# uingei/hevc

Hardware: AMD Instinct MI355X
Metric: encoded 1080p30 frames/sec/GPU; PSNR-Y parity vs libx265 at matched bitrate (higher is better)
Workload: dtype u8

## Files before the change

hevc_amd/csrc/device.hip:

```cpp
#include "device.h"
#include "md5.h"

#include <cstdio>
#include <cstring>
#include <vector>

namespace mihevc {

__host__ __device__ static inline size_t round16(size_t v) { return (v + 15) & ~(size_t)15; }

__device__ __forceinline__ int xcd_remap(int b, int n)
{
    int chunk = (n + 7) >> 3;
    return (b & 7) * chunk + (b >> 3);
}

template <typename T> __global__ __launch_bounds__(NT, 5) void k_me_search(const InterArgs<T> *args, int n_ctu, int list)
{
    extern __shared__ __align__(16) unsigned char smem[];
    const int ctu = xcd_remap(blockIdx.x, n_ctu);
    if (ctu >= n_ctu) return;
    MeShared<T> &s = *reinterpret_cast<MeShared<T> *>(smem);
    uint8_t *win = smem + round16(sizeof(MeShared<T>));
    GpuExec ex;
    if (list) {
        const InterArgs<T> a = list1_view(args[blockIdx.y]);
        me_search_program<T>(ex, s, win, a, ctu);
    } else me_search_program<T>(ex, s, win, args[blockIdx.y], ctu);
}

template <typename T> __global__ __launch_bounds__(NT, 4) void k_inter_ctu(const InterArgs<T> *args, int n_ctu)
{
    extern __shared__ __align__(16) unsigned char smem[];
    const int ctu = xcd_remap(blockIdx.x, n_ctu);
    if (ctu >= n_ctu) return;
    const InterArgs<T> &a = args[blockIdx.y];
    const int R = a.prm.me_range;
    InterShared<T> &s = *reinterpret_cast<InterShared<T> *>(smem);
    size_t off = round16(sizeof(InterShared<T>));
    T *wy = reinterpret_cast<T *>(smem + off);
    off += round16(((size_t)mc_win_y(R) * mc_win_y_stride(R) + 16) * sizeof(T));
    T *wu = reinterpret_cast<T *>(smem + off);
    off += round16(((size_t)mc_win_c(R) * mc_win_c_stride(R) + 16) * sizeof(T));
    T *wv = reinterpret_cast<T *>(smem + off);
    GpuExec ex;
    inter_ctu_program<T>(ex, s, wy, wu, wv, a, ctu);
}

template <typename T> __global__ __launch_bounds__(NT, 3) void k_inter_ctu_b(const InterArgs<T> *args, int n_ctu)
{
    extern __shared__ __align__(16) unsigned char smem[];
    const int ctu = xcd_remap(blockIdx.x, n_ctu);
    if (ctu >= n_ctu) return;
    const InterArgs<T> &a = args[blockIdx.y];
    const int R = a.prm.me_range;
    InterShared<T> &s = *reinterpret_cast<InterShared<T> *>(smem);
    size_t off = round16(sizeof(InterShared<T>));
    T *wy = reinterpret_cast<T *>(smem + off);
    off += round16(((size_t)mc_win_y(R) * mc_win_y_stride(R) + 16) * sizeof(T));
    T *wu = reinterpret_cast<T *>(smem + off);
    off += round16(((size_t)mc_win_c(R) * mc_win_c_stride(R) + 16) * sizeof(T));
    T *wv = reinterpret_cast<T *>(smem + off);
    off += round16(((size_t)mc_win_c(R) * mc_win_c_stride(R) + 16) * sizeof(T));
    BiShared *b = reinterpret_cast<BiShared *>(smem + off);
    GpuExec ex;
    inter_ctu_program<T, GpuExec, true>(ex, s, wy, wu, wv, a, ctu, b);
}

#ifndef INTRA_OCC
#define INTRA_OCC 3
#endif
template <typename T> __global__ __launch_bounds__(NT, (sizeof(T) == 1 ? INTRA_OCC : 2)) void k_intra_plan(const IntraArgs<T> *args, int n_ctu)
{
    extern __shared__ __align__(16) unsigned char smem[];
    const int ctu = xcd_remap(blockIdx.x, n_ctu);
    if (ctu >= n_ctu) return;
    const IntraArgs<T> &a = args[blockIdx.y];
    IntraShared<T> &s = *reinterpret_cast<IntraShared<T> *>(smem);
    GpuExec ex;
    intra_plan_program<T>(ex, s, a, ctu % a.ctus_w, ctu / a.ctus_w);
}

template <typename T> __global__ __launch_bounds__(NT, 2) void k_intra_diag(const IntraArgs<T> *args, int diagonal, int rows_per_tile)
{
    extern __shared__ __align__(16) unsigned char smem[];
    const IntraArgs<T> &a = args[blockIdx.y];
    const int tcn = a.prm.tile_cols > 1 ? a.prm.tile_cols : 1, trn = a.prm.tile_rows > 1 ? a.prm.tile_rows : 1;
    const int tile = (int)blockIdx.x / rows_per_tile, r = (int)blockIdx.x % rows_per_tile;
    if (tile >= tcn * trn) return;
    const int tx = tile % tcn, ty = tile / tcn;
    const int cx0 = tile_bd(tx, tcn, a.ctus_w), cx1 = tile_bd(tx + 1, tcn, a.ctus_w), cy0 = tile_bd(ty, trn, a.ctus_h), cy1 = tile_bd(ty + 1, trn, a.ctus_h);
    const int cy = cy0 + r, cx = cx0 + diagonal - 2 * r;
    if (cy >= cy1 || cx < cx0 || cx >= cx1) return;
    IntraShared<T> &s = *reinterpret_cast<IntraShared<T> *>(smem);
    GpuExec ex;
    intra_code_program<T>(ex, s, a, cx, cy, true);
}

template <typename T> __global__ __launch_bounds__(256) void k_lowres(const PreArgs<T> *args)
// ... 209 lines not shown
        i -= ncp;
        if (i < ncp) pad_border_quad<T>(a.out[2], a.w >> 1, a.h >> 1, PAD_C, i, a.halo_top >> 1, a.halo_bottom >> 1);
        return;
    }
    b -= n_pad_blocks;
    if (b < n_low_blocks) { lowres_sample<T>(pre[g], b * 256 + (int)threadIdx.x); return; }
    if (threadIdx.x == 0) {
        CostParams c = p.prm[g];
        ea[g].prm = c; sa[g].prm = c;
        c.tile_cols = p.p_tile_cols; c.tile_rows = p.p_tile_rows;
        ia[g].prm = c;
    }
    if (threadIdx.x < 4) sa[g].sse[threadIdx.x] = 0;
}

template <typename T> hipError_t launch_prep_p_step(hipStream_t st, const SaoArgs<T> *prev, const PreArgs<T> *pre, IntraArgs<T> *ia, InterArgs<T> *ea, SaoArgs<T> *sa,
                                                    const StepParams &p, int w, int h, int batch)
{
    if (batch > MAX_LANES) return hipErrorInvalidValue;
    const int n_pad = prev ? (pad_border_quads(w, h, PAD_Y) + 2 * pad_border_quads(w >> 1, h >> 1, PAD_C) + 255) / 256 : 0;
    const int n_low = pre ? (2 * (w >> 2) * (h >> 2) + 255) / 256 : 0;
    hipLaunchKernelGGL(k_prep_p_step<T>, dim3((unsigned)(n_pad + n_low + 1), (unsigned)batch), dim3(256), 0, st, prev, n_pad, pre, n_low, ia, ea, sa, p);
    return hipGetLastError();
}
template <typename T> hipError_t launch_begin_p_step(hipStream_t st, IntraArgs<T> *ia, InterArgs<T> *ea, SaoArgs<T> *sa, const StepParams &p, int batch)
{
    if (batch > MAX_LANES) return hipErrorInvalidValue;
    hipLaunchKernelGGL(k_begin_p_step<T>, dim3((unsigned)batch), dim3(64), 0, st, ia, ea, sa, p);
    return hipGetLastError();
}
template <typename T> hipError_t launch_frame_sse(hipStream_t st, const SaoArgs<T> *d_args, int batch)
{
    hipLaunchKernelGGL(k_frame_sse<T>, dim3(256, (unsigned)batch), dim3(256), 0, st, d_args);
    return hipGetLastError();
}
template <typename K> static hipError_t ensure_smem(K kernel, size_t bytes)
{
    if (bytes <= 48 * 1024) return hipSuccess;
    return hipFuncSetAttribute(reinterpret_cast<const void *>(kernel), hipFuncAttributeMaxDynamicSharedMemorySize, (int)bytes);
}

template <typename T> hipError_t launch_me_search(hipStream_t st, const InterArgs<T> *d_args, int n_ctu, int batch, int R, int list)
{
    size_t smem = round16(sizeof(MeShared<T>)) + round16((size_t)me_win_elems(R));
    hipError_t e = ensure_smem(k_me_search<T>, smem);
    if (e != hipSuccess) return e;
    dim3 grid((unsigned)(((n_ctu + 7) >> 3) << 3), (unsigned)batch);
    hipLaunchKernelGGL(k_me_search<T>, grid, dim3(NT), smem, st, d_args, n_ctu, list);
    return hipGetLastError();
}

template <typename T> hipError_t launch_inter_ctu(hipStream_t st, const InterArgs<T> *d_args, int n_ctu, int batch, int R)
{
    size_t smem = round16(sizeof(InterShared<T>)) + round16(((size_t)mc_win_y(R) * mc_win_y_stride(R) + 16) * sizeof(T)) +
                  2 * round16(((size_t)mc_win_c(R) * mc_win_c_stride(R) + 16) * sizeof(T));
    hipError_t e = ensure_smem(k_inter_ctu<T>, smem);
    if (e != hipSuccess) return e;
    dim3 grid((unsigned)(((n_ctu + 7) >> 3) << 3), (unsigned)batch);
    hipLaunchKernelGGL(k_inter_ctu<T>, grid, dim3(NT), smem, st, d_args, n_ctu);
    return hipGetLastError();
}

template <typename T> hipError_t launch_inter_ctu_b(hipStream_t st, const InterArgs<T> *d_args, int n_ctu, int batch, int R)
{
    size_t smem = round16(sizeof(InterShared<T>)) + round16(((size_t)mc_win_y(R) * mc_win_y_stride(R) + 16) * sizeof(T)) +
                  2 * round16(((size_t)mc_win_c(R) * mc_win_c_stride(R) + 16) * sizeof(T)) + round16(sizeof(BiShared));
    hipError_t e = ensure_smem(k_inter_ctu_b<T>, smem);
    if (e != hipSuccess) return e;
    dim3 grid((unsigned)(((n_ctu + 7) >> 3) << 3), (unsigned)batch);
    hipLaunchKernelGGL(k_inter_ctu_b<T>, grid, dim3(NT), smem, st, d_args, n_ctu);
    return hipGetLastError();
}

template <typename T> hipError_t launch_intra_picture(hipStream_t st, const IntraArgs<T> *d_args, int ctus_w, int ctus_h, int batch, int tile_cols, int tile_rows, hipEvent_t after_plan)
{
    size_t smem = round16(sizeof(IntraShared<T>));
    hipError_t e = ensure_smem(k_intra_plan<T>, smem);
    if (e != hipSuccess) return e;
    e = ensure_smem(k_intra_diag<T>, smem);
    if (e != hipSuccess) return e;
    if (tile_cols < 1) tile_cols = 1;
    if (tile_rows < 1) tile_rows = 1;
    const int n_ctu = ctus_w * ctus_h;
    hipLaunchKernelGGL(k_intra_plan<T>, dim3((unsigned)(((n_ctu + 7) >> 3) << 3), (unsigned)batch), dim3(NT), smem, st, d_args, n_ctu);
    if (after_plan) { e = hipEventRecord(after_plan, st); if (e != hipSuccess) return e; }
    const int colw = (ctus_w + tile_cols - 1) / tile_cols, rowh = (ctus_h + tile_rows - 1) / tile_rows;
    for (int d = 0; d <= (colw - 1) + 2 * (rowh - 1); d++)
        hipLaunchKernelGGL(k_intra_diag<T>, dim3((unsigned)(tile_cols * tile_rows * rowh), (unsigned)batch), dim3(NT), smem, st, d_args, d, rowh);
    return hipGetLastError();
}

template <typename T> hipError_t launch_pre_search(hipStream_t st, const PreArgs<T> *d_args, int w, int h, int n_ctu, int batch, bool with_lowres)
{
    const int n = 2 * (w >> 2) * (h >> 2);
    if (with_lowres) hipLaunchKernelGGL(k_lowres<T>, dim3((unsigned)((n + 255) / 256), (unsigned)batch), dim3(256), 0, st, d_args);
    hipLaunchKernelGGL(k_pre_search<T>, dim3((unsigned)n_ctu, (unsigned)batch), dim3(NT), 0, st, d_args, n_ctu);
    return hipGetLastError();
}

template <typename T> __global__ __launch_bounds__(256) void k_lowres_src(const PreArgs<T> *args)
{
    const PreArgs<T> &a = args[blockIdx.y];
    const int i = (int)(blockIdx.x * 256 + threadIdx.x);
    if (i < (a.w >> 2) * (a.h >> 2)) lowres_sample<T>(a, i);
}
template <typename T> hipError_t launch_pre_search_chunk(hipStream_t st, const PreArgs<T> *d_args, int w, int h, int n_ctu, int n_pictures)
{
    if (n_pictures <= 0) return hipSuccess;
    const int n = (w >> 2) * (h >> 2);
    hipLaunchKernelGGL(k_lowres_src<T>, dim3((unsigned)((n + 255) / 256), (unsigned)n_pictures), dim3(256), 0, st, d_args);
    hipLaunchKernelGGL(k_pre_search<T>, dim3((unsigned)n_ctu, (unsigned)n_pictures), dim3(NT), 0, st, d_args, n_ctu);
    return hipGetLastError();
// ... 558 lines not shown
```

hevc_amd/csrc/kernels/common.h:

```cpp
#pragma once
#include <stdint.h>

#if defined(__HIPCC__)
#include <hip/hip_runtime.h>
#define DEV __device__ __forceinline__
#define HD __host__ __device__
#define HDI __host__ __device__ inline
#define DEVCONST __device__ const
#define MIHEVC_GPU 1
#else
#define DEV inline
#define HD
#define HDI inline
#define DEVCONST static const
#define MIHEVC_GPU 0
#endif

#include "../../../include/mihevc.h"

namespace mihevc {

constexpr int CTU = 32;
constexpr int CTU_LOG2 = 5;
constexpr int PAD_Y = 80;
// ... 237 lines not shown
DEV void copy_window(T *lds, int ls, const T *plane, int pstride, int ox, int oy, int w, int h, int lo_x, int hi_x, int lo_y, int hi_y, int tid)
{
    constexpr int per = 4 / (int)sizeof(T);
    constexpr int CH = 6;
    const int dpr = w / per, col = tid & 31, rg = tid >> 5;
    for (int d = col; d < dpr; d += 32) {
        const int x = clip3(lo_x, hi_x - (per - 1), ox + d * per);
        for (int r0 = rg; r0 < h; r0 += CH * (NT / 32)) {
            uint32_t v[CH];
#pragma unroll
            for (int k = 0; k < CH; k++) {
                const int r = r0 + k * (NT / 32);
                if (r < h) v[k] = load_u32(plane + (ptrdiff_t)clip3(lo_y, hi_y, oy + r) * pstride + x);
            }
#pragma unroll
            for (int k = 0; k < CH; k++) {
                const int r = r0 + k * (NT / 32);
                if (r < h) __builtin_memcpy(__builtin_assume_aligned(lds + r * ls + d * per, 4), &v[k], 4);
            }
        }
    }
}

template <typename T>
DEV void load_ctu_source(T *dst, const Plane<const T> (&src)[3], int x0, int y0, int w, int h, int tid)
{
    constexpr int per = 4 / (int)sizeof(T);
    if (x0 + CTU <= w && y0 + CTU <= h) {
        constexpr int ND = 1536 / per, IT = (ND + NT - 1) / NT;
        uint32_t v[IT];
#pragma unroll
        for (int k = 0; k < IT; k++) {
            const int d = tid + k * NT;
            if (d < ND) {
                const int i = d * per, pl = i < 1024 ? 0 : 1 + ((i - 1024) >> 8), kk = pl ? (i - 1024) & 255 : i, x = pl ? kk & 15 : kk & 31, y = pl ? kk >> 4 : kk >> 5;
                v[k] = load_u32(src[pl].p + (size_t)((pl ? y0 >> 1 : y0) + y) * src[pl].stride + (pl ? x0 >> 1 : x0) + x);
            }
        }
#pragma unroll
        for (int k = 0; k < IT; k++) {
            const int d = tid + k * NT;
            if (d < ND) __builtin_memcpy(__builtin_assume_aligned(dst + d * per, 4), &v[k], 4);
        }
        return;
    }
    for (int i = tid; i < 1536; i += NT) {
        int pl, x, y;
        if (i < 1024) { pl = 0; x = i & 31; y = i >> 5; } else { int k = i - 1024; pl = 1 + (k >> 8); k &= 255; x = k & 15; y = k >> 4; }
        const int gx = (pl ? x0 >> 1 : x0) + x, gy = (pl ? y0 >> 1 : y0) + y, pw = pl ? w >> 1 : w, ph = pl ? h >> 1 : h;
        dst[i] = (gx < pw && gy < ph) ? src[pl].p[(size_t)gy * src[pl].stride + gx] : (T)0;
    }
}

DEV int opaque_zero()
{
    int z = 0;
#if MIHEVC_GPU
    asm volatile("" : "+v"(z));
#endif
    return z;
}
DEV uint32_t load_u32_aligned(const void *p)
{
    uint32_t v;
    __builtin_memcpy(&v, __builtin_assume_aligned(p, 4), 4);
    return v;
}
DEV void store_u32_aligned(void *p, uint32_t v) { __builtin_memcpy(__builtin_assume_aligned(p, 4), &v, 4); }
DEV void store4(uint8_t *p, int v0, int v1, int v2, int v3) { store_u32_aligned(p, (uint32_t)v0 | (uint32_t)v1 << 8 | (uint32_t)v2 << 16 | (uint32_t)v3 << 24); }
DEV void store4(uint16_t *p, int v0, int v1, int v2, int v3)
{
    store_u32_aligned(p, (uint32_t)v0 | (uint32_t)v1 << 16);
    store_u32_aligned(p + 2, (uint32_t)v2 | (uint32_t)v3 << 16);
}
DEV void store4(int16_t *p, int v0, int v1, int v2, int v3)
{
    store_u32_aligned(p, ((uint32_t)v0 & 0xffffu) | (uint32_t)v1 << 16);
    store_u32_aligned(p + 2, ((uint32_t)v2 & 0xffffu) | (uint32_t)v3 << 16);
}
DEV void load_row15(const uint8_t *base, int idx, int (&px)[15])
{
    const int off = idx & 3;
    const uint8_t *p = base + (idx - off);
    uint32_t d[5];
#pragma unroll
    for (int k = 0; k < 5; k++) d[k] = load_u32_aligned(p + 4 * k);
    uint32_t r[4];
#pragma unroll
    for (int k = 0; k < 4; k++) r[k] = align_bytes(d[k + 1], d[k], off);
#pragma unroll
    for (int i = 0; i < 15; i++) px[i] = (int)((r[i >> 2] >> (8 * (i & 3))) & 255);
}
DEV void load_row15(const uint16_t *base, int idx, int (&px)[15])
{
    const int off = idx & 1;
    const uint16_t *p = base + (idx - off);
    uint32_t d[8];
#pragma unroll
    for (int k = 0; k < 8; k++) d[k] = load_u32_aligned(p + 2 * k);
    uint32_t r[8];
#pragma unroll
    for (int k = 0; k < 7; k++) r[k] = align_bytes(d[k + 1], d[k], 2 * off);
    r[7] = align_bytes(0, d[7], 2 * off);
#pragma unroll
    for (int i = 0; i < 15; i++) px[i] = (int)((r[i >> 1] >> (16 * (i & 1))) & 65535);
}
// ... 89 lines not shown
    int s = 0;
#pragma unroll
    for (int x = 0; x < 8; x++) {
#pragma unroll
        for (int st = 1; st < 8; st <<= 1)
#pragma unroll
            for (int i = 0; i < 8; i++)
                if (!(i & st)) { int p = m[i][x], q = m[i + st][x]; m[i][x] = p + q; m[i + st][x] = p - q; }
#pragma unroll
        for (int i = 0; i < 8; i++) if (x || i) s += iabs(m[i][x]);
    }
    return (s + 2) >> 2;
}

#if MIHEVC_GPU
#ifdef MIHEVC_PHASE_PROF
__device__ unsigned long long g_phase_prof[8 * 1024 * 3];
#endif
struct GpuExec {
    static DEV int lane_id()
    {
        int t = (int)threadIdx.x;
        asm volatile("" : "+v"(t));
        return t;
    }
#ifdef MIHEVC_PHASE_PROF
    template <class F> DEV void phase(F &&f, int line = __builtin_LINE(), const char *file = __builtin_FILE())
    {
        int len = 0;
        while (file[len]) len++;
        const int fid = ((int)file[len - 3] + 2 * (int)file[len - 4] + 3 * (int)file[len - 6]) & 7;
        const int slot = (fid * 1024 + (line & 1023)) * 3;
        const unsigned long long t0 = __builtin_amdgcn_s_memtime();
        f(lane_id());
        const unsigned long long t1 = __builtin_amdgcn_s_memtime();
        __syncthreads();
        if (threadIdx.x == 0) {
            const unsigned long long t2 = __builtin_amdgcn_s_memtime();
            atomicAdd(&g_phase_prof[slot], t2 - t0);
            atomicAdd(&g_phase_prof[slot + 1], t1 - t0);
            atomicAdd(&g_phase_prof[slot + 2], 1ull);
        }
    }
#else
    template <class F> DEV void phase(F &&f)
    {
        f(lane_id());
        __syncthreads();
    }
#endif
    template <class F> DEV void wave_step(F &&f)
    {
        f(lane_id());
        __builtin_amdgcn_fence(__ATOMIC_SEQ_CST, "wavefront");
        __builtin_amdgcn_wave_barrier();
    }
    DEV void atomic_add(int *p, int v) { atomicAdd(p, v); }
    DEV void atomic_add(unsigned *p, unsigned v) { atomicAdd(p, v); }
    DEV void atomic_add(unsigned long long *p, unsigned long long v) { atomicAdd(p, v); }
    DEV void atomic_or(unsigned *p, unsigned v) { atomicOr(p, v); }
    DEV void atomic_and(unsigned *p, unsigned v) { atomicAnd(p, v); }
    DEV void atomic_min(unsigned long long *p, unsigned long long v) { atomicMin(p, v); }
    DEV unsigned long long peek(const unsigned long long *p) { return __atomic_load_n(p, __ATOMIC_RELAXED); }
    DEV void atomic_add_global(unsigned long long *p, unsigned long long v) { atomicAdd(p, v); }
};
#endif
struct SeqExec {
    int order = 0;
    unsigned long long rnd = 0x2545F4914F6CDD1Dull;
    template <class F> void run(F &&f)
    {
        if (order == 0) { for (int t = 0; t < NT; t++) f(t); return; }
        if (order == 1) { for (int t = NT - 1; t >= 0; t--) f(t); return; }
        int perm[NT];
        for (int i = 0; i < NT; i++) perm[i] = i;
        for (int i = NT - 1; i > 0; i--) {
            rnd ^= rnd << 13; rnd ^= rnd >> 7; rnd ^= rnd << 17;
            int j = (int)((rnd >> 33) % (unsigned)(i + 1)), tmp = perm[i];
            perm[i] = perm[j]; perm[j] = tmp;
        }
        for (int i = 0; i < NT; i++) f(perm[i]);
    }
    template <class F> void phase(F &&f) { run(f); }
    template <class F> void wave_step(F &&f) { run(f); }
    void atomic_add(int *p, int v) { *p += v; }
    void atomic_add(unsigned *p, unsigned v) { *p += v; }
    void atomic_add(unsigned long long *p, unsigned long long v) { *p += v; }
    void atomic_or(unsigned *p, unsigned v) { *p |= v; }
    void atomic_and(unsigned *p, unsigned v) { *p &= v; }
    void atomic_min(unsigned long long *p, unsigned long long v) { if (v < *p) *p = v; }
    unsigned long long peek(const unsigned long long *p) { return *p; }
    void atomic_add_global(unsigned long long *p, unsigned long long v) { *p += v; }
};

}
```

hevc_amd/csrc/kernels/inter.h:

```cpp
#pragma once
#include "common.h"
#include "residual.h"

namespace mihevc {

template <typename T> struct InterArgs {
    Plane<const T> src[3];
    Plane<const T> ref[3];
    Plane<T> rec[3];
    int w, h, ctus_w;
    CostParams prm;
    const int16_t *centers;
    int32_t *me;
    mihevc_cu_rec *cu;
    int16_t *coef[3];
    unsigned long long *est;
    int sparse_coef;
    IpInfo *ip;
    Plane<const T> ref1[3];
    const int16_t *centers1;
    int32_t *me1;
};
template <typename T> DEV InterArgs<T> list1_view(const InterArgs<T> &a)
{
// ... 279 lines not shown
                    const int br = half * 2 + r2;
                    unsigned o[4][4];
                    quad_block_row(srcp + br * 8 * 32, win + (br * 8 + dyi) * ws + 4 * q, ws, o);
#pragma unroll
                    for (int b = 0; b < 4; b++) {
#pragma unroll
                        for (int j = 0; j < 4; j++) s16[b >> 1][j] += o[b][j];
                        consider(5 + (half * 2 + (b >> 1)) * 4 + r2 * 2 + (b & 1), o[b]);
                    }
                }
#pragma unroll
                for (int h2 = 0; h2 < 2; h2++) {
#pragma unroll
                    for (int j = 0; j < 4; j++) s32[j] += s16[h2][j];
                    consider(1 + half * 2 + h2, s16[h2]);
                }
            }
            consider(0, s32);
        }
    });
    ex.phase([&](int tid) {
        if (tid < 21) {
            int32_t *o = a.me + ((size_t)ctu * 21 + tid) * 3;
            if (s.valid[tid]) {
                int p = (int)(s.best[tid] & 0xffff);
                o[0] = 4 * (sx + p % spanx - R); o[1] = 4 * (sy + p / spanx - R); o[2] = (int32_t)(s.best[tid] >> 16);
            } else { o[0] = 0; o[1] = 0; o[2] = -1; }
        }
    });
}

template <typename T> struct InterShared {
    ResidualShared rs;
    T src[1536];
    T pred[1536];
    int mvx[21], mvy[21];
    unsigned cost[21];
    uint8_t valid[21];
    int satd[3][1][16];
    unsigned nsum[21];
    unsigned fsum[8][21];
    unsigned long long rbest[21];
    unsigned j16[4];
    int use16[4], use32;
    uint8_t alias[3][16];
    int tile_mvx[16], tile_mvy[16];
    uint8_t tile_node[16];
    uint8_t chosen[21];
    unsigned est;
    unsigned ip_cost, ip_act, ip_tiles;
    unsigned long long ip_sse;
    unsigned tu_dc[3][16], tu_dz[3][16], tu_bits[3][16], tu_zero[3];
};
HDI int mc_win_y(int R) { return (32 + 2 * (R + 3) + 8 + 3) & ~3; }
HDI int mc_win_y_stride(int R) { return mc_win_y(R) + 4; }
HDI int mc_win_c(int R) { return (16 + (R + 3) + 8 + 3) & ~3; }
HDI int mc_win_c_stride(int R) { return mc_win_c(R) + 4; }

template <typename T>
DEV int luma_tile(const T *win, int i00, int ws, int fx, int fy, int bit_depth, const T *diff_src, int src_stride, T *pred_out, int pred_stride)
{
    const int8_t *tx = g_tab.luma_tap[fx], *ty = g_tab.luma_tap[fy];
    const int shift1 = bit_depth - 8, shift3 = 14 - bit_depth, maxv = (1 << bit_depth) - 1;
    int acc[8][8];
#pragma unroll
    for (int j = 0; j < 8; j++)
#pragma unroll
        for (int i = 0; i < 8; i++) acc[j][i] = 0;
    for (int r = 0; r < 15; r++) {
        int px[15];
        load_row15(win, i00 + (r - 3) * ws - 3, px);
        int hv[8];
#pragma unroll
        for (int i = 0; i < 8; i++) {
            int v = 0;
#pragma unroll
            for (int k = 0; k < 8; k++) v += tx[k] * px[i + k];
            hv[i] = v >> shift1;
        }
#pragma unroll
        for (int j = 0; j < 8; j++) {
            int k = r - j;
            if (k >= 0 && k < 8) {
                int t = ty[k];
#pragma unroll
                for (int i = 0; i < 8; i++) acc[j][i] += t * hv[i];
            }
        }
    }
    const int off = 1 << (shift3 - 1);
#pragma unroll
    for (int j = 0; j < 8; j++)
#pragma unroll
        for (int i = 0; i < 8; i++) {
            int v = clip3(0, maxv, ((acc[j][i] >> 6) + off) >> shift3);
            if (diff_src) acc[j][i] = (int)diff_src[j * src_stride + i] - v;
            else pred_out[j * pred_stride + i] = (T)v;
        }
    return diff_src ? hadamard8_satd(acc) : 0;
}

DEV int luma_tile(const uint8_t *win, int i00, int ws, int fx, int fy, int bit_depth, const uint8_t *diff_src, int src_stride, uint8_t *pred_out,
                  int pred_stride)
{
    const uint32_t tlo = load_u32(&g_tab.luma_tap[fx][0]), thi = load_u32(&g_tab.luma_tap[fx][4]);
    uint32_t typ[4];
#pragma unroll
    for (int m = 0; m < 4; m++) typ[m] = pack_lo16(g_tab.luma_tap[fy][2 * m], g_tab.luma_tap[fy][2 * m + 1]);
    int acc[8][8], prev[8];
#pragma unroll
// ... 359 lines not shown
    return clip3(0, maxv, ((acc >> 6) + (1 << (shift3 - 1))) >> shift3);
}

template <typename T> DEV void luma_quad14(const T *win, int i00, int ws, int fx, int fy, int bit_depth, int (&out)[4])
{
    const int8_t *tx = g_tab.luma_tap[fx], *ty = g_tab.luma_tap[fy];
    const int shift1 = bit_depth - 8;
    int acc[4] = {0, 0, 0, 0};
#pragma unroll
    for (int r = 0; r < 8; r++) {
        int px[15];
        load_row15(win, i00 + (r - 3) * ws - 3, px);
        const int t = ty[r];
#pragma unroll
        for (int i = 0; i < 4; i++) {
            int v = 0;
#pragma unroll
            for (int k = 0; k < 8; k++) v += tx[k] * px[i + k];
            acc[i] += t * (v >> shift1);
        }
    }
#pragma unroll
    for (int i = 0; i < 4; i++) out[i] = acc[i] >> 6;
}
template <typename T> DEV int chroma_sample14(const T *p00, int ws, int fx, int fy, int bit_depth)
{
    const int8_t *tx = g_tab.chroma_tap[fx], *ty = g_tab.chroma_tap[fy];
    const int shift1 = bit_depth - 8;
    int acc = 0;
    for (int r = 0; r < 4; r++) {
        const T *row = p00 + (r - 1) * ws - 1;
        int v = tx[0] * row[0] + tx[1] * row[1] + tx[2] * row[2] + tx[3] * row[3];
        acc += ty[r] * (v >> shift1);
    }
    return acc >> 6;
}
DEV int weighted_uni(int p, int bit_depth) { const int sh = 14 - bit_depth; return clip3(0, (1 << bit_depth) - 1, (p + (1 << (sh - 1))) >> sh); }
DEV int weighted_bi(int p0, int p1, int bit_depth) { const int sh = 15 - bit_depth; return clip3(0, (1 << bit_depth) - 1, (p0 + p1 + (1 << (sh - 1))) >> sh); }
struct BiShared {
    int mx0[21], my0[21];
    unsigned c0[21], cb[21];
    uint8_t mode[21];
    uint8_t tile_mode[16];
    int tile_mv1x[16], tile_mv1y[16];
    alignas(16) int16_t p0[1536];
};

template <typename T, class Ex, bool BI = false>
DEV void inter_ctu_program(Ex &ex, InterShared<T> &s, T *win_y, T *win_u, T *win_v, const InterArgs<T> &a, int ctu, BiShared *bsh = nullptr)
{
    const int R0 = a.prm.me_range, R = R0 + 3, bd = a.prm.bit_depth, lam = a.prm.lambda_sad_q4;
    const int x0 = (ctu % a.ctus_w) * CTU, y0 = (ctu / a.ctus_w) * CTU;
    const int mct = a.prm.mc_top, mcb = a.prm.mc_bottom;
    const int sx = a.centers ? a.centers[2 * ctu] : 0, sy0 = a.centers ? a.centers[2 * ctu + 1] : 0;
    const int sy = (mct || mcb) ? clamp_center_y(sy0, y0, R0, a.h, mct, mcb) : sy0;
    const int wy = mc_win_y(R0), wys = mc_win_y_stride(R0), wc = mc_win_c(R0), wcs = mc_win_c_stride(R0);
    const int oy_x = x0 + sx - R - 4, oy_y = y0 + sy - R - 4;
    const int oc_x = (x0 >> 1) + ((4 * sx - 4 * R - 3) >> 3) - 1, oc_y = (y0 >> 1) + ((4 * sy - 4 * R - 3) >> 3) - 1;

    ex.phase([&](int tid) {
        residual_init_lane(s.rs, tid);
        load_ctu_source<T>(s.src, a.src, x0, y0, a.w, a.h, tid);
        copy_window<T>(win_y, wys, a.ref[0].p, a.ref[0].stride, oy_x, oy_y, wy, wy, -PAD_Y, a.w + PAD_Y - 1, -PAD_Y, a.h + PAD_Y - 1, tid);
        copy_window<T>(win_u, wcs, a.ref[1].p, a.ref[1].stride, oc_x, oc_y, wc, wc, -PAD_C, (a.w >> 1) + PAD_C - 1, -PAD_C, (a.h >> 1) + PAD_C - 1, tid);
        copy_window<T>(win_v, wcs, a.ref[2].p, a.ref[2].stride, oc_x, oc_y, wc, wc, -PAD_C, (a.w >> 1) + PAD_C - 1, -PAD_C, (a.h >> 1) + PAD_C - 1, tid);
        if (tid < 21) {
            const int32_t *m = a.me + ((size_t)ctu * 21 + tid) * 3;
            s.mvx[tid] = m[0]; s.mvy[tid] = m[1]; s.valid[tid] = m[2] >= 0; s.cost[tid] = 0; s.nsum[tid] = 0;
        }
    });
    ex.phase([&](int tid) {
        for (int u = tid; u < 3 * 16; u += NT) {
            int level = u >> 4, t = u & 15;
            int txp = t & 3, typ = t >> 2, node = node_of_tile(level, txp, typ);
            if (!s.valid[node]) continue;
            int al = level;
            for (int fl = 2; fl > level; fl--) {
                int fn = node_of_tile(fl, txp, typ);
                if (s.valid[fn] && s.mvx[fn] == s.mvx[node] && s.mvy[fn] == s.mvy[node]) { al = fl; break; }
            }
            s.alias[level][t] = (uint8_t)al;
            if (al != level) continue;
            int px = x0 + txp * 8 + (s.mvx[node] >> 2) - oy_x, py = y0 + typ * 8 + (s.mvy[node] >> 2) - oy_y;
            s.satd[level][0][t] = luma_tile_int<T>(win_y, py * wys + px, wys, s.src + typ * 8 * 32 + txp * 8, 32);
        }
    });
    ex.phase([&](int tid) {
        if (tid < 3 * 16) {
            const int level = tid >> 4, t = tid & 15, node = node_of_tile(level, t & 3, t >> 2);
            if (s.valid[node]) ex.atomic_add(&s.nsum[node], (unsigned)s.satd[s.alias[level][t]][0][t]);
        }
        if (tid >= 64 && tid < 64 + 8 * 21) s.fsum[(tid - 64) / 21][(tid - 64) % 21] = 0;
    });
    ex.wave_step([&](int tid) {
        if (tid >= 21) return;
        s.chosen[tid] = 0;
        s.cost[tid] = s.valid[tid] ? (s.nsum[tid] << 4) + (unsigned)(lam * (mvd_bits(s.mvx[tid] - 4 * sx) + mvd_bits(s.mvy[tid] - 4 * sy))) : 0;
        if (tid == 0) { s.est = 0; s.ip_cost = 0; s.ip_act = 0; s.ip_tiles = 0; s.ip_sse = 0; }
    });
    ex.wave_step([&](int tid) {
        if (tid >= 4) return;
        const int q = tid;
        unsigned js = (unsigned)(lam * 2);
        for (int t = 0; t < 4; t++) if (s.valid[5 + 4 * q + t]) js += s.cost[5 + 4 * q + t] + (unsigned)(lam * 4);
        const unsigned jw = s.cost[1 + q] + (unsigned)(lam * 4);
        s.use16[q] = s.valid[1 + q] && jw <= js;
        s.j16[q] = s.use16[q] ? jw : js;
    });
    ex.wave_step([&](int tid) {
        if (tid != 0) return;
        const unsigned js32 = (unsigned)(lam * 2) + s.j16[0] + s.j16[1] + s.j16[2] + s.j16[3];
        s.use32 = s.valid[0] && s.cost[0] + (unsigned)(lam * 4) <= js32;
    });
    ex.phase([&](int tid) {
        if (tid >= 16) return;
        const int t = tid, txp = t & 3, typ = t >> 2, q = (typ >> 1) * 2 + (txp >> 1), n8 = node_of_tile(2, txp, typ);
        const int node = s.use32 ? 0 : s.use16[q] ? 1 + q : n8, inside = s.valid[n8];
        s.tile_node[t] = (uint8_t)node;
        if (inside) s.chosen[node] = 1;
        s.rs.tu_log2[t] = inside ? (uint8_t)(node == 0 ? 5 : node < 5 ? 4 : 3) : 0;
        s.rs.tu_intra[t] = 0;
    });
    auto refine = [&](const int csx, const int csy, const int wox, const int woy) {
    for (int round = 0; round < 2; round++) {
        const int step = round == 0 ? 2 : 1;
        ex.wave_step([&](int tid) {
            const int u = tid >> 1, half = tid & 1, k = kRingSlot[u >> 4], t = u & 15;
            if (!s.rs.tu_log2[t]) return;
            const int txp = t & 3, typ = t >> 2, node = s.tile_node[t];
            const int mx = s.mvx[node] + kOff[k][0] * step, my = s.mvy[node] + kOff[k][1] * step;
            const int px = x0 + txp * 8 + 4 * half + (mx >> 2) - wox, py = y0 + typ * 8 + (my >> 2) - woy;
            int m[8][4];
            luma_half_diff((const T *)win_y, py * wys + px, wys, mx & 3, my & 3, bd, (const T *)(s.src + typ * 8 * 32 + txp * 8 + 4 * half), 32, m);
            {
                uint32_t P[4][4];
#pragma unroll
                for (int r2 = 0; r2 < 4; r2++)
#pragma unroll
                    for (int c = 0; c < 4; c++) P[r2][c] = perm_bytes((uint32_t)m[2 * r2 + 1][c], (uint32_t)m[2 * r2][c], 0x05040100u);
#pragma unroll
                for (int c = 0; c < 4; c++) {
                    const uint32_t a0 = pk_add16(P[0][c], P[1][c]), a1 = pk_sub16(P[0][c], P[1][c]), a2 = pk_add16(P[2][c], P[3][c]), a3 = pk_sub16(P[2][c], P[3][c]);
                    P[0][c] = pk_add16(a0, a2); P[1][c] = pk_add16(a1, a3); P[2][c] = pk_sub16(a0, a2); P[3][c] = pk_sub16(a1, a3);
                }
                uint32_t *x = s.rs.scratch + tid * 16;
                const int sw = tid >> 2;
#pragma unroll
                for (int r2 = 0; r2 < 4; r2++) {
                    const uint32_t p0 = pk_add16(P[r2][0], P[r2][1]), p1 = pk_sub16(P[r2][0], P[r2][1]), p2 = pk_add16(P[r2][2], P[r2][3]), p3 = pk_sub16(P[r2][2], P[r2][3]);
                    const uint32_t o[4] = {pk_add16(p0, p2), pk_add16(p1, p3), pk_sub16(p0, p2), pk_sub16(p1, p3)};
                    store_x4(x + 4 * ((r2 + sw) & 3), o);
                }
            }
        });
        ex.wave_step([&](int tid) {
            const int u = tid >> 1, half = tid & 1, t = u & 15;
            if (!s.rs.tu_log2[t]) return;
            const uint32_t *xa = s.rs.scratch + (tid & ~1) * 16, *xb = xa + 16;
            const int sw = tid >> 2;
            unsigned sum = 0;
            {
                uint32_t acc[2] = {0, 0};
#pragma unroll
                for (int c = 0; c < 2; c++) {
                    uint32_t va[4], vb[4];
                    const int at = 4 * ((2 * half + c + sw) & 3);
                    load_x4(xa + at, va); load_x4(xb + at, vb);
#pragma unroll
                    for (int i = 0; i < 4; i++) {
#pragma unroll
                        for (int sgn = 0; sgn < 2; sgn++) {
                            const uint32_t v = sgn ? pk_sub16(va[i], vb[i]) : pk_add16(va[i], vb[i]);
                            const uint32_t av = pk_max_i16(v, pk_sub16(0u, v));
                            const uint32_t mx = pk_max_i16(av, (av >> 16) | (av << 16));
                            if constexpr (sizeof(T) == 1) acc[c] = pk_add16(acc[c], mx); else sum += mx & 0xffffu;
                        }
                    }
                }
                if constexpr (sizeof(T) == 1) sum = (acc[0] & 0xffffu) + (acc[1] & 0xffffu);
                s.rs.scratch[4096 + tid] = 2u * sum;
            }
        });
        ex.phase([&](int tid) {
            const int u = tid >> 1, k = kRingSlot[u >> 4], t = u & 15;
            if (tid >= 1 && tid < 43 && (tid & 1)) s.rbest[tid >> 1] = (unsigned long long)s.cost[tid >> 1] << 4;
            if ((tid & 1) || !s.rs.tu_log2[t]) return;
            const unsigned satd = (s.rs.scratch[4096 + tid] + s.rs.scratch[4096 + tid + 1] + 2) >> 2;
            ex.atomic_add(&s.fsum[k - 1][s.tile_node[t]], satd);
        });
        ex.phase([&](int tid) {
            const int node = tid >> 3, k = 1 + (tid & 7);
            if (node >= 21 || !s.valid[node] || !s.chosen[node]) return;
            const unsigned satd = s.fsum[k - 1][node];
            s.fsum[k - 1][node] = 0;
            const int mx = s.mvx[node] + kOff[k][0] * step, my = s.mvy[node] + kOff[k][1] * step;
            if (mct || mcb) {
                int nx, ny, nl;
                node_geom(node, nx, ny, nl);
                if (!mv_rows_ok(y0 + ny, 1 << nl, my, a.h, mct, mcb)) return;
            }
            const unsigned c = (satd << 4) + (unsigned)(lam * (mvd_bits(mx - 4 * csx) + mvd_bits(my - 4 * csy)));
            ex.atomic_min(&s.rbest[node], ((unsigned long long)c << 4) | (unsigned)k);
        });
        ex.phase([&](int tid) {
            if (tid >= 21 || !s.valid[tid] || !s.chosen[tid]) return;
            const unsigned long long best = s.rbest[tid];
            const int k = (int)(best & 15);
            s.mvx[tid] += kOff[k][0] * step; s.mvy[tid] += kOff[k][1] * step;
            s.cost[tid] = (unsigned)(best >> 4);
        });
    }
    };
    refine(sx, sy, oy_x, oy_y);
    if constexpr (BI) {
        BiShared &b = *bsh;
        const int sx1 = a.centers1 ? a.centers1[2 * ctu] : 0, sy1 = a.centers1 ? a.centers1[2 * ctu + 1] : 0;
        const int o1_x = x0 + sx1 - R - 4, o1_y = y0 + sy1 - R - 4;
        const int oc1_x = (x0 >> 1) + ((4 * sx1 - 4 * R - 3) >> 3) - 1, oc1_y = (y0 >> 1) + ((4 * sy1 - 4 * R - 3) >> 3) - 1;
        ex.phase([&](int tid) {
            if (tid < 21) { b.mx0[tid] = s.mvx[tid]; b.my0[tid] = s.mvy[tid]; b.c0[tid] = s.cost[tid]; b.cb[tid] = 0; }
            {
                const int t = tid >> 4, j = (tid >> 1) & 7, hx = (tid & 1) * 4, txp = t & 3, typ = t >> 2;
                if (s.rs.tu_log2[t]) {
                    const int node = s.tile_node[t], mx = s.mvx[node], my = s.mvy[node];
                    const int px = x0 + txp * 8 + hx + (mx >> 2) - oy_x, py = y0 + typ * 8 + j + (my >> 2) - oy_y;
                    int v[4];
                    luma_quad14<T>(win_y, py * wys + px, wys, mx & 3, my & 3, bd, v);
#pragma unroll
                    for (int i = 0; i < 4; i++) b.p0[(typ * 8 + j) * 32 + txp * 8 + hx + i] = (int16_t)v[i];
                }
            }
            for (int i = tid; i < 512; i += NT) {
                const int pl = i >> 8, k = i & 255, x = k & 15, y = k >> 4, t = (y >> 2) * 4 + (x >> 2);
                if (!s.rs.tu_log2[t]) continue;
                const int node = s.tile_node[t], mx = s.mvx[node], my = s.mvy[node];
                const int px = (x0 >> 1) + x + (mx >> 3) - oc_x, py = (y0 >> 1) + y + (my >> 3) - oc_y;
                b.p0[1024 + i] = (int16_t)chroma_sample14<T>((pl ? win_v : win_u) + py * wcs + px, wcs, mx & 7, my & 7, bd);
            }
        });
        ex.phase([&](int tid) {
// ... 239 lines not shown
```

Baseline: 5354.

## Shrink inter-CTU LDS footprint by packing MC windows into residual scratch

```diff
diff --git a/hevc_amd/csrc/device.hip b/hevc_amd/csrc/device.hip
--- a/hevc_amd/csrc/device.hip
+++ b/hevc_amd/csrc/device.hip
@@ -29,22 +29,17 @@
     } else me_search_program<T>(ex, s, win, args[blockIdx.y], ctu);
 }
 
-template <typename T> __global__ __launch_bounds__(NT, 4) void k_inter_ctu(const InterArgs<T> *args, int n_ctu)
+template <typename T, bool Y_IN> __global__ __launch_bounds__(NT, (sizeof(T) == 1 ? 5 : 4)) void k_inter_ctu(const InterArgs<T> *args, int n_ctu)
 {
     extern __shared__ __align__(16) unsigned char smem[];
     const int ctu = xcd_remap(blockIdx.x, n_ctu);
     if (ctu >= n_ctu) return;
     const InterArgs<T> &a = args[blockIdx.y];
-    const int R = a.prm.me_range;
+    const InterLds l = inter_lds<T>(a.prm.me_range);
     InterShared<T> &s = *reinterpret_cast<InterShared<T> *>(smem);
-    size_t off = round16(sizeof(InterShared<T>));
-    T *wy = reinterpret_cast<T *>(smem + off);
-    off += round16(((size_t)mc_win_y(R) * mc_win_y_stride(R) + 16) * sizeof(T));
-    T *wu = reinterpret_cast<T *>(smem + off);
-    off += round16(((size_t)mc_win_c(R) * mc_win_c_stride(R) + 16) * sizeof(T));
-    T *wv = reinterpret_cast<T *>(smem + off);
-    GpuExec ex;
-    inter_ctu_program<T>(ex, s, wy, wu, wv, a, ctu);
+    T *wy = reinterpret_cast<T *>(smem + (Y_IN ? inter_win_in<T>() : inter_win_out<T>()));
+    GpuExec ex;
+    inter_ctu_program<T>(ex, s, wy, reinterpret_cast<T *>(smem + l.u), reinterpret_cast<T *>(smem + l.v), a, ctu);
 }
 
 template <typename T> __global__ __launch_bounds__(NT, 3) void k_inter_ctu_b(const InterArgs<T> *args, int n_ctu)
@@ -360,12 +355,12 @@
 
 template <typename T> hipError_t launch_inter_ctu(hipStream_t st, const InterArgs<T> *d_args, int n_ctu, int batch, int R)
 {
-    size_t smem = round16(sizeof(InterShared<T>)) + round16(((size_t)mc_win_y(R) * mc_win_y_stride(R) + 16) * sizeof(T)) +
-                  2 * round16(((size_t)mc_win_c(R) * mc_win_c_stride(R) + 16) * sizeof(T));
-    hipError_t e = ensure_smem(k_inter_ctu<T>, smem);
+    const InterLds l = inter_lds<T>(R);
+    auto kernel = l.y == inter_win_in<T>() ? k_inter_ctu<T, true> : k_inter_ctu<T, false>;
+    hipError_t e = ensure_smem(kernel, l.bytes);
     if (e != hipSuccess) return e;
     dim3 grid((unsigned)(((n_ctu + 7) >> 3) << 3), (unsigned)batch);
-    hipLaunchKernelGGL(k_inter_ctu<T>, grid, dim3(NT), smem, st, d_args, n_ctu);
+    hipLaunchKernelGGL(kernel, grid, dim3(NT), l.bytes, st, d_args, n_ctu);
     return hipGetLastError();
 }
 
diff --git a/hevc_amd/csrc/kernels/common.h b/hevc_amd/csrc/kernels/common.h
--- a/hevc_amd/csrc/kernels/common.h
+++ b/hevc_amd/csrc/kernels/common.h
@@ -313,6 +313,13 @@
     }
 }
 
+DEV int wave_uniform(int v)
+{
+#if MIHEVC_GPU
+    v = __builtin_amdgcn_readfirstlane(v);
+#endif
+    return v;
+}
 DEV int opaque_zero()
 {
     int z = 0;
@@ -508,6 +515,10 @@
     template <class F> DEV void wave_step(F &&f)
     {
         f(lane_id());
+        wave_sync();
+    }
+    static DEV void wave_sync()
+    {
         __builtin_amdgcn_fence(__ATOMIC_SEQ_CST, "wavefront");
         __builtin_amdgcn_wave_barrier();
     }
@@ -520,7 +531,20 @@
     DEV unsigned long long peek(const unsigned long long *p) { return __atomic_load_n(p, __ATOMIC_RELAXED); }
     DEV void atomic_add_global(unsigned long long *p, unsigned long long v) { atomicAdd(p, v); }
 };
-#endif
+template <class F, class... G> DEV void wave_chain(GpuExec &, F &&first, G &&...then)
+{
+    const int tid = GpuExec::lane_id();
+    auto st = first(tid);
+    GpuExec::wave_sync();
+    ((then(tid, st), GpuExec::wave_sync()), ...);
+}
+#endif
+template <class Ex, class F, class... G> DEV void wave_chain(Ex &ex, F &&first, G &&...then)
+{
+    decltype(first(0)) st[NT];
+    ex.wave_step([&](int tid) { st[tid] = first(tid); });
+    (ex.wave_step([&](int tid) { then(tid, st[tid]); }), ...);
+}
 struct SeqExec {
     int order = 0;
     unsigned long long rnd = 0x2545F4914F6CDD1Dull;
diff --git a/hevc_amd/csrc/kernels/inter.h b/hevc_amd/csrc/kernels/inter.h
--- a/hevc_amd/csrc/kernels/inter.h
+++ b/hevc_amd/csrc/kernels/inter.h
@@ -355,10 +355,29 @@
     unsigned long long ip_sse;
     unsigned tu_dc[3][16], tu_dz[3][16], tu_bits[3][16], tu_zero[3];
 };
+constexpr int FRAC_PAIR_SUM = 8 * NT;
+constexpr int FRAC_SCRATCH = FRAC_PAIR_SUM + NT;
+static_assert(FRAC_SCRATCH <= (int)(sizeof(ResidualShared::scratch) / 4), "the fractional search's exchange must fit rs.scratch");
 HDI int mc_win_y(int R) { return (32 + 2 * (R + 3) + 8 + 3) & ~3; }
 HDI int mc_win_y_stride(int R) { return mc_win_y(R) + 4; }
 HDI int mc_win_c(int R) { return (16 + (R + 3) + 8 + 3) & ~3; }
 HDI int mc_win_c_stride(int R) { return mc_win_c(R) + 4; }
+
+struct InterLds { size_t y, u, v, bytes; };
+template <typename T> HDI constexpr size_t inter_win_in() { return offsetof(InterShared<T>, rs) + offsetof(ResidualShared, scratch) + 4 * (size_t)FRAC_SCRATCH; }
+template <typename T> HDI constexpr size_t inter_win_out() { return (sizeof(InterShared<T>) + 15) & ~(size_t)15; }
+template <typename T> HDI InterLds inter_lds(int R)
+{
+    const size_t n[3] = {((size_t)mc_win_y(R) * mc_win_y_stride(R) + 16) * sizeof(T), ((size_t)mc_win_c(R) * mc_win_c_stride(R) + 16) * sizeof(T),
+                         ((size_t)mc_win_c(R) * mc_win_c_stride(R) + 16) * sizeof(T)};
+    const size_t hi = offsetof(InterShared<T>, rs) + offsetof(ResidualShared, scratch) + sizeof(ResidualShared::scratch);
+    size_t in = inter_win_in<T>(), out = inter_win_out<T>(), at[3];
+    for (int i = 0; i < 3; i++) {
+        const size_t r = (n[i] + 15) & ~(size_t)15;
+        if (in + r <= hi) { at[i] = in; in += r; } else { at[i] = out; out += r; }
+    }
+    return InterLds{at[0], at[1], at[2], out};
+}
 
 template <typename T>
 DEV int luma_tile(const T *win, int i00, int ws, int fx, int fy, int bit_depth, const T *diff_src, int src_stride, T *pred_out, int pred_stride)
@@ -824,7 +843,7 @@
     const int R0 = a.prm.me_range, R = R0 + 3, bd = a.prm.bit_depth, lam = a.prm.lambda_sad_q4;
     const int x0 = (ctu % a.ctus_w) * CTU, y0 = (ctu / a.ctus_w) * CTU;
     const int mct = a.prm.mc_top, mcb = a.prm.mc_bottom;
-    const int sx = a.centers ? a.centers[2 * ctu] : 0, sy0 = a.centers ? a.centers[2 * ctu + 1] : 0;
+    const int sx = wave_uniform(a.centers ? a.centers[2 * ctu] : 0), sy0 = wave_uniform(a.centers ? a.centers[2 * ctu + 1] : 0);
     const int sy = (mct || mcb) ? clamp_center_y(sy0, y0, R0, a.h, mct, mcb) : sy0;
     const int wy = mc_win_y(R0), wys = mc_win_y_stride(R0), wc = mc_win_c(R0), wcs = mc_win_c_stride(R0);
     const int oy_x = x0 + sx - R - 4, oy_y = y0 + sy - R - 4;
@@ -896,9 +915,11 @@
     auto refine = [&](const int csx, const int csy, const int wox, const int woy) {
     for (int round = 0; round < 2; round++) {
         const int step = round == 0 ? 2 : 1;
-        ex.wave_step([&](int tid) {
+        struct Kept { uint32_t v[2][4]; };
+        wave_chain(ex, [&](int tid) -> Kept {
             const int u = tid >> 1, half = tid & 1, k = kRingSlot[u >> 4], t = u & 15;
-            if (!s.rs.tu_log2[t]) return;
+            Kept kept{};
+            if (!s.rs.tu_log2[t]) return kept;
             const int txp = t & 3, typ = t >> 2, node = s.tile_node[t];
             const int mx = s.mvx[node] + kOff[k][0] * step, my = s.mvy[node] + kOff[k][1] * step;
             const int px = x0 + txp * 8 + 4 * half + (mx >> 2) - wox, py = y0 + typ * 8 + (my >> 2) - woy;
@@ -915,29 +936,36 @@
                     const uint32_t a0 = pk_add16(P[0][c], P[1][c]), a1 = pk_sub16(P[0][c], P[1][c]), a2 = pk_add16(P[2][c], P[3][c]), a3 = pk_sub16(P[2][c], P[3][c]);
                     P[0][c] = pk_add16(a0, a2); P[1][c] = pk_add16(a1, a3); P[2][c] = pk_sub16(a0, a2); P[3][c] = pk_sub16(a1, a3);
                 }
-                uint32_t *x = s.rs.scratch + tid * 16;
-                const int sw = tid >> 2;
+                uint32_t o[4][4];
 #pragma unroll
                 for (int r2 = 0; r2 < 4; r2++) {
                     const uint32_t p0 = pk_add16(P[r2][0], P[r2][1]), p1 = pk_sub16(P[r2][0], P[r2][1]), p2 = pk_add16(P[r2][2], P[r2][3]), p3 = pk_sub16(P[r2][2], P[r2][3]);
-                    const uint32_t o[4] = {pk_add16(p0, p2), pk_add16(p1, p3), pk_sub16(p0, p2), pk_sub16(p1, p3)};
-                    store_x4(x + 4 * ((r2 + sw) & 3), o);
-                }
-            }
-        });
-        ex.wave_step([&](int tid) {
-            const int u = tid >> 1, half = tid & 1, t = u & 15;
+                    o[r2][0] = pk_add16(p0, p2); o[r2][1] = pk_add16(p1, p3); o[r2][2] = pk_sub16(p0, p2); o[r2][3] = pk_sub16(p1, p3);
+                }
+                uint32_t *x = s.rs.scratch + tid * 8;
+                const int sw = ((tid >> 2) ^ (tid >> 3)) & 1;
+#pragma unroll
+                for (int c = 0; c < 2; c++) {
+                    uint32_t send[4];
+#pragma unroll
+                    for (int i = 0; i < 4; i++) { kept.v[c][i] = half ? o[2 + c][i] : o[c][i]; send[i] = half ? o[c][i] : o[2 + c][i]; }
+                    store_x4(x + 4 * (c ^ sw), send);
+                }
+            }
+            return kept;
+        }, [&](int tid, const Kept &kept) {
+            const int u = tid >> 1, t = u & 15;
             if (!s.rs.tu_log2[t]) return;
-            const uint32_t *xa = s.rs.scratch + (tid & ~1) * 16, *xb = xa + 16;
-            const int sw = tid >> 2;
+            const uint32_t *xp = s.rs.scratch + (tid ^ 1) * 8;
+            const int sw = ((tid >> 2) ^ (tid >> 3)) & 1;
             unsigned sum = 0;
             {
                 uint32_t acc[2] = {0, 0};
 #pragma unroll
                 for (int c = 0; c < 2; c++) {
-                    uint32_t va[4], vb[4];
-                    const int at = 4 * ((2 * half + c + sw) & 3);
-                    load_x4(xa + at, va); load_x4(xb + at, vb);
+                    uint32_t vb[4];
+                    load_x4(xp + 4 * (c ^ sw), vb);
+                    const uint32_t (&va)[4] = kept.v[c];
 #pragma unroll
                     for (int i = 0; i < 4; i++) {
 #pragma unroll
@@ -950,14 +978,14 @@
                     }
                 }
                 if constexpr (sizeof(T) == 1) sum = (acc[0] & 0xffffu) + (acc[1] & 0xffffu);
-                s.rs.scratch[4096 + tid] = 2u * sum;
+                s.rs.scratch[FRAC_PAIR_SUM + tid] = 2u * sum;
             }
         });
         ex.phase([&](int tid) {
             const int u = tid >> 1, k = kRingSlot[u >> 4], t = u & 15;
             if (tid >= 1 && tid < 43 && (tid & 1)) s.rbest[tid >> 1] = (unsigned long long)s.cost[tid >> 1] << 4;
             if ((tid & 1) || !s.rs.tu_log2[t]) return;
-            const unsigned satd = (s.rs.scratch[4096 + tid] + s.rs.scratch[4096 + tid + 1] + 2) >> 2;
+            const unsigned satd = (s.rs.scratch[FRAC_PAIR_SUM + tid] + s.rs.scratch[FRAC_PAIR_SUM + tid + 1] + 2) >> 2;
             ex.atomic_add(&s.fsum[k - 1][s.tile_node[t]], satd);
         });
         ex.phase([&](int tid) {
```

Measured after the change: 5613 (median of 6 runs). +4.8%, better.
